# ngrabaskas/Torch-Automatic-Distributed-Neural-Network

Hardware: AMD Instinct MI355X
Metric: samples/sec whole-node ResNet-50 DP + GPT-2 PP at 1/2/4/8 MI355X; scaling eff (higher is better)
Workload: dtype bf16

## Files before the change

### madnn/ops/csrc/stem.hip

```cpp
#include "mfma.h"

namespace madnn {
namespace stem {

using namespace mf;

constexpr int kThreads = 256;
constexpr int kCo = 64;
constexpr int kKh = 7;
constexpr int kKp = 224;
constexpr int kSteps = kKp / 16;
constexpr int kMaxWo = 128;

struct StemArgs {
  const uint16_t* x;
  const uint16_t* w;
  uint16_t* y;
  float* stats;
  int N, H, W, Ho, Wo;
  int rows;
};

__device__ __forceinline__ int img_elem(int kh, int px, int c, int WP) { return (kh * WP + px) * 4 + c; }

template <bool STATS>
__global__ __launch_bounds__(kThreads, 2) void stem_fwd_kernel(const StemArgs a) {
  extern __shared__ __attribute__((aligned(16))) uint16_t smem[];
  const int WP = 2 * a.Wo + 6;
  const int IMG = kKh * WP * 4;
  uint16_t* img0 = smem;
  uint16_t* img1 = smem + IMG;
  char* otile = reinterpret_cast<char*>(smem + 2 * IMG);
  const int tid = threadIdx.x, wave = tid >> 6, lane = tid & 63, l32 = lane & 31, hh = lane >> 5;
  const int row_elems = a.W * 3;
  const int chunks = (row_elems + 7) / 8;
  const int PER = (kKh * chunks + kThreads - 1) / kThreads;

  for (int i = tid; i < IMG; i += kThreads) {
    img0[i] = 0;
    img1[i] = 0;
  }

  const int nb = wave & 1, pb0 = 64 * (wave >> 1);
  bf16x8 wf[kSteps];
#pragma unroll
  for (int s = 0; s < kSteps; ++s)
    wf[s] = *reinterpret_cast<const bf16x8*>(a.w + (32 * nb + l32) * kKp + 16 * s + 8 * hh);

  float ssum[8], ssq[8];
  if constexpr (STATS) {
#pragma unroll
    for (int e = 0; e < 8; ++e) ssum[e] = ssq[e] = 0.f;
  }

  u32x4 stg[4];
  auto load = [&](int row) {
    const int n = row / a.Ho, oh = row % a.Ho;
#pragma unroll
    for (int i = 0; i < 4; ++i) {
      const int c = tid + kThreads * i;
      stg[i] = u32x4{0u, 0u, 0u, 0u};
      if (i < PER && c < kKh * chunks) {
        const int kh = c / chunks, ch = c % chunks;
        const int ih = 2 * oh - 3 + kh;
        if (ih >= 0 && ih < a.H) {
          stg[i] = *reinterpret_cast<const u32x4*>(a.x + ((int64_t)n * a.H + ih) * row_elems + ch * 8);
        }
      }
    }
  };
  auto store = [&](uint16_t* img) {
#pragma unroll
    for (int i = 0; i < 4; ++i) {
      const int c = tid + kThreads * i;
      if (i < PER && c < kKh * chunks) {
        const int kh = c / chunks, ch = c % chunks;
#pragma unroll
        for (int k = 0; k < 8; ++k) {
          const int e = ch * 8 + k;
          const unsigned v = (stg[i][k >> 1] >> (16 * (k & 1))) & 0xffffu;
          img[img_elem(kh, e / 3 + 3, e % 3, WP)] = (uint16_t)v;
        }
      }
    }
  };

  int row = blockIdx.x;
  if (row >= a.rows) return;
  __syncthreads();
  load(row);
  store(img0);
  __syncthreads();
  int cur = 0;
  for (;;) {
    const int nrow = row + gridDim.x;
    const bool more = nrow < a.rows;
    if (more) load(nrow);
    const uint16_t* img = cur ? img1 : img0;
    f32x16 acc[2] = {zero16(), zero16()};
    if (pb0 < a.Wo) {
#pragma unroll
      for (int kh = 0; kh < kKh; ++kh)
#pragma unroll
        for (int s2 = 0; s2 < 2; ++s2) {
#pragma unroll
          for (int q = 0; q < 2; ++q) {
            const int pix = min(pb0 + 32 * q + l32, a.Wo - 1);
            const int px = 2 * pix + 4 * s2 + 2 * hh;
            const bf16x8 bx = *reinterpret_cast<const bf16x8*>(img + img_elem(kh, px, 0, WP));
            acc[q] = mfma(wf[2 * kh + s2], bx, acc[q]);
          }
        }
    }
#pragma unroll
    for (int q = 0; q < 2; ++q) {
      const int pix = pb0 + 32 * q + l32;
#pragma unroll
      for (int g = 0; g < 4; ++g) {
        const int co = 32 * nb + 8 * g + 4 * hh;
        const unsigned lo = (unsigned)f32_to_bf16(acc[q][4 * g]) | ((unsigned)f32_to_bf16(acc[q][4 * g + 1]) << 16);
        const unsigned hi = (unsigned)f32_to_bf16(acc[q][4 * g + 2]) | ((unsigned)f32_to_bf16(acc[q][4 * g + 3]) << 16);
        *reinterpret_cast<u32x2*>(otile + pix * 128 + 16 * ((co >> 3) ^ ((pix >> 1) & 7)) + 8 * ((co >> 2) & 1)) =
            u32x2{lo, hi};
      }
    }
    __syncthreads();
    {
      uint16_t* yrow = a.y + (int64_t)row * a.Wo * kCo;
      const int c = tid & 7;
      for (int r = tid >> 3; r < a.Wo; r += kThreads / 8) {
        const u32x4 v = *reinterpret_cast<const u32x4*>(otile + r * 128 + 16 * (c ^ ((r >> 1) & 7)));
        *reinterpret_cast<u32x4*>(yrow + r * kCo + 8 * c) = v;
        if constexpr (STATS) {
#pragma unroll
          for (int e = 0; e < 4; ++e) {
            const float x0 = bf16_to_f32((unsigned short)(v[e] & 0xffffu));
            const float x1 = bf16_to_f32((unsigned short)(v[e] >> 16));
            ssum[2 * e] += x0;
            ssq[2 * e] += x0 * x0;
            ssum[2 * e + 1] += x1;
            ssq[2 * e + 1] += x1 * x1;
          }
        }
      }
    }
    if (!more) break;
    store(cur ? img0 : img1);
    __syncthreads();
    cur ^= 1;
    row = nrow;
  }

  if constexpr (STATS) {
    __syncthreads();
    float* red = reinterpret_cast<float*>(otile);
    const int c = tid & 7, rg = tid >> 3;
#pragma unroll
    for (int e = 0; e < 8; ++e) {
      red[(rg * 2) * kCo + 8 * c + e] = ssum[e];
      red[(rg * 2 + 1) * kCo + 8 * c + e] = ssq[e];
    }
    __syncthreads();
    if (tid < 2 * kCo) {
      const int which = tid / kCo, co = tid % kCo;
      float v = 0.f;
      for (int g = 0; g < kThreads / 8; ++g) v += red[(g * 2 + which) * kCo + co];
      a.stats[((int64_t)blockIdx.x * 2 + which) * kCo + co] = v;
    }
  }
}

inline int stem_grid(int rows) { return rows < 2 * kNumCU ? rows : 2 * kNumCU; }

constexpr int kWMaxTiles = 4;

struct StemWArgs {
  const uint16_t* x;
  const uint16_t* dy;
  float* ws;
  int N, H, W, Ho, Wo;
  int rows, per;
  const uint16_t* y;
  const uint16_t* dp;
  const uint64_t* arg;
  const float* sc;
  const float* sh;
  const float* ca;
  const float* cb;
  const float* cc;
  int Hp, Wp, p;
};

__device__ __forceinline__ bf16x8 lds_patch(const uint16_t* img_row, int ow0, int lane) {
  const int g = lane >> 4, i = lane & 15;
  const int kw = 4 * (g & 1) + (i & 3);
  const int ow = ow0 + 8 * (g >> 1) + (i >> 2);
  typedef __attribute__((address_space(3))) s16x4 lds_s16x4;
  const uint16_t* p = img_row + (2 * ow + kw) * 4;
  const s16x4 lo = __builtin_amdgcn_ds_read_tr16_b64_v4i16((lds_s16x4*)p);
  const s16x4 hi = __builtin_amdgcn_ds_read_tr16_b64_v4i16((lds_s16x4*)(p + 8 * 4));
  const s16x8 r = {lo[0], lo[1], lo[2], lo[3], hi[0], hi[1], hi[2], hi[3]};
  return __builtin_bit_cast(bf16x8, r);
}

template <bool BNP>
__global__ __launch_bounds__(kThreads, 2) void stem_wgrad_kernel(const StemWArgs a) {
  extern __shared__ __attribute__((aligned(16))) uint16_t smem[];
  const int WOP = (a.Wo + 15) & ~15;
  const int ROW = (2 * WOP + 6) * 4;
  uint16_t* ring = smem;
  uint16_t* dyt = smem + 9 * ROW;
  const int pchunks = BNP ? a.Wp * 8 : 0;
  uint16_t* pdp = dyt + WOP * kCo;
  uint64_t* parg = reinterpret_cast<uint64_t*>(pdp + 2 * pchunks * 8);
  float* cf = reinterpret_cast<float*>(parg + 2 * pchunks);
  int tid = threadIdx.x;
  const int wave = tid >> 6, lane = tid & 63, hh = lane >> 5, l32 = lane & 31;
  const int row_elems = a.W * 3, chunks = row_elems / 8;
  const int dchunks = a.Wo * 8;

  const int r0 = blockIdx.x * a.per;
  const int r1 = min(r0 + a.per, a.rows);
  if (r0 >= r1) return;
  for (int i = tid; i < 9 * ROW + WOP * kCo; i += kThreads) smem[i] = 0;

  const int b = wave & 1, kh0 = wave >> 1;
  f32x16 acc[kWMaxTiles];
#pragma unroll
  for (int q = 0; q < kWMaxTiles; ++q) acc[q] = zero16();

  u32x4 istg[4], dstg[4];
  int s_oh = 0, s_klo = 0;
  u32x4 pstg[2];
  u32x2 astg[2];
  int s_pslot = -1;
  auto pload = [&](int n, int ohp) {
    if constexpr (BNP) asm volatile("" : "+v"(tid));
    s_pslot = ohp & 1;
    const int64_t base = ((int64_t)n * a.Hp + ohp) * pchunks;
#pragma unroll
    for (int i = 0; i < 2; ++i) {
      const int c = tid + kThreads * i;
      if (c < pchunks) {
        pstg[i] = *reinterpret_cast<const u32x4*>(a.dp + (base + c) * 8);
        astg[i] = *reinterpret_cast<const u32x2*>(a.arg + base + c);
      }
    }
  };
  auto pstore = [&]() {
    if (s_pslot < 0) return;
    if constexpr (BNP) asm volatile("" : "+v"(tid));
#pragma unroll
    for (int i = 0; i < 2; ++i) {
      const int c = tid + kThreads * i;
      if (c < pchunks) {
        *reinterpret_cast<u32x4*>(pdp + (s_pslot * pchunks + c) * 8) = pstg[i];
        *reinterpret_cast<u32x2*>(parg + s_pslot * pchunks + c) = astg[i];
      }
    }
  };
  auto load = [&](int r) {
    if constexpr (BNP) asm volatile("" : "+v"(tid));
    const int n = r / a.Ho, oh = r % a.Ho;
    const bool fresh = (r == r0) || (oh == 0);
    s_oh = oh;
    s_klo = fresh ? 0 : 5;
    if constexpr (BNP) {
      const int h1 = (oh + a.p) >> 1;
      s_pslot = -1;
      if ((fresh || ((oh + a.p) & 1) == 0) && h1 < a.Hp) pload(n, h1);
    }
    const int total = (kKh - s_klo) * chunks;
#pragma unroll
    for (int i = 0; i < 4; ++i) {
      const int c = tid + kThreads * i;
      istg[i] = u32x4{0u, 0u, 0u, 0u};
      if (c < total) {
        const int ih = 2 * oh - 3 + s_klo + c / chunks;
        if (ih >= 0 && ih < a.H)
          istg[i] = *reinterpret_cast<const u32x4*>(a.x + ((int64_t)n * a.H + ih) * row_elems + (c % chunks) * 8);
      }
      const int d = tid + kThreads * i;
      if (d < dchunks)
        dstg[i] = *reinterpret_cast<const u32x4*>((BNP ? a.y : a.dy) + ((int64_t)r * a.Wo) * kCo + d * 8);
    }
  };
  auto store = [&]() {
    if constexpr (BNP) asm volatile("" : "+v"(tid));
    const int total = (kKh - s_klo) * chunks;
#pragma unroll
    for (int i = 0; i < 4; ++i) {
      const int c = tid + kThreads * i;
      if (c < total) {
        const int ih = 2 * s_oh - 3 + s_klo + c / chunks, ch = c % chunks;
        if (ih >= 0 && ih < a.H) {
          uint16_t* img = ring + (ih & 7) * ROW;
#pragma unroll
          for (int k = 0; k < 8; ++k) {
            const int e = ch * 8 + k;
            img[(e / 3 + 3) * 4 + e % 3] = (uint16_t)((istg[i][k >> 1] >> (16 * (k & 1))) & 0xffffu);
          }
        }
      }
      if constexpr (!BNP) {
        const int d = tid + kThreads * i;
        if (d < dchunks)
          *reinterpret_cast<u32x4*>(reinterpret_cast<char*>(dyt) + swz<64>(d >> 3, d & 7)) = dstg[i];
      }
    }
    if constexpr (BNP) pstore();
  };
  auto build = [&]() {
    const int hp = s_oh + a.p, h1 = hp >> 1, hodd = hp & 1;
    const bool okh[2] = {hodd == 0 && h1 >= 1, h1 < a.Hp};
    if constexpr (BNP) asm volatile("" : "+v"(tid));
    const int cg = tid & 7;
    float v[5][8];
#pragma unroll
    for (int k = 0; k < 5; ++k) {
      const f32x4 lo = *reinterpret_cast<const f32x4*>(cf + k * kCo + cg * 8);
      const f32x4 hi = *reinterpret_cast<const f32x4*>(cf + k * kCo + cg * 8 + 4);
      v[k][0] = lo.x; v[k][1] = lo.y; v[k][2] = lo.z; v[k][3] = lo.w;
      v[k][4] = hi.x; v[k][5] = hi.y; v[k][6] = hi.z; v[k][7] = hi.w;
    }
#pragma unroll
    for (int i = 0; i < 4; ++i) {
      const int d = tid + kThreads * i;
      if (d < dchunks) {
        const int wp = (d >> 3) + a.p, w1 = wp >> 1, wodd = wp & 1;
        const bool okw[2] = {wodd == 0 && w1 >= 1, w1 < a.Wp};
        u32x4 g[4];
        u32x2 pk[4];
        bool ok[4];
        unsigned pos[4];
#pragma unroll
        for (int q = 0; q < 4; ++q) {
          const int ih = q >> 1, iw = q & 1;
          ok[q] = okh[ih] && okw[iw];
          pos[q] = (unsigned)((ih ? hodd : 2) * 3 + (iw ? wodd : 2));
          const int ow = min(max(w1 - 1 + iw, 0), a.Wp - 1);
          const int c = (((h1 - 1 + ih) & 1) * a.Wp + ow) * 8 + cg;
          g[q] = *reinterpret_cast<const u32x4*>(pdp + c * 8);
          pk[q] = *reinterpret_cast<const u32x2*>(parg + c);
        }
        u32x4 o4;
#pragma unroll
        for (int j2 = 0; j2 < 4; ++j2) {
          unsigned short ob[2];
#pragma unroll
          for (int e = 0; e < 2; ++e) {
            const int j = 2 * j2 + e;
            float acc = 0.f;
#pragma unroll
            for (int q = 0; q < 4; ++q) {
              const float gj = bf16_to_f32((unsigned short)((g[q][j >> 1] >> (16 * (j & 1))) & 0xffffu));
              const unsigned byte = (pk[q][j >> 2] >> (8 * (j & 3))) & 0xffu;
              if (ok[q]) acc += (byte == pos[q]) ? gj : 0.f;
            }
            const float yv = bf16_to_f32((unsigned short)((dstg[i][j >> 1] >> (16 * (j & 1))) & 0xffffu));
            const float z = yv * v[0][j] + v[1][j];
            acc = z > 0.f ? acc : 0.f;
            ob[e] = f32_to_bf16(v[2][j] * acc + v[3][j] * yv + v[4][j]);
          }
          o4[j2] = (unsigned)ob[0] | ((unsigned)ob[1] << 16);
        }
        *reinterpret_cast<u32x4*>(reinterpret_cast<char*>(dyt) + swz<64>(d >> 3, d & 7)) = o4;
      }
      __builtin_amdgcn_sched_barrier(0);
    }
  };

  if constexpr (BNP) {
    for (int i = tid; i < 5 * kCo; i += kThreads) {
      const float* src = i < kCo ? a.sc : i < 2 * kCo ? a.sh : i < 3 * kCo ? a.ca : i < 4 * kCo ? a.cb : a.cc;
      cf[i] = src[i % kCo];
    }
  }
  __syncthreads();
  if constexpr (BNP) {
    const int n = r0 / a.Ho, hp = r0 % a.Ho + a.p;
    if ((hp & 1) == 0 && (hp >> 1) >= 1) {
      pload(n, (hp >> 1) - 1);
      pstore();
    }
  }
  load(r0);
  store();
  __syncthreads();
  if constexpr (BNP) {
    build();
    __syncthreads();
  }
  for (int r = r0;;) {
    const int oh = r % a.Ho;
    const bool more = r + 1 < r1;
    if (more) load(r + 1);
    const uint16_t* rows_kh[kWMaxTiles];
#pragma unroll
    for (int q = 0; q < kWMaxTiles; ++q) {
      const int ih = 2 * oh - 3 + kh0 + 2 * q;
      rows_kh[q] = ring + ((ih >= 0 && ih < a.H) ? (ih & 7) : 8) * ROW;
    }
    for (int t = 0; t < WOP; t += 16) {
      const bf16x8 af = lds_col<64>(dyt, t, 32 * b, lane);
#pragma unroll
      for (int q = 0; q < kWMaxTiles; ++q)
        if (kh0 + 2 * q < kKh) acc[q] = mfma(af, lds_patch(rows_kh[q], t, lane), acc[q]);
    }
    if (!more) break;
    __syncthreads();
    store();
    __syncthreads();
    if constexpr (BNP) {
      build();
      __syncthreads();
    }
    ++r;
  }

  const int kw = l32 >> 2, c = l32 & 3;
  if (kw < 7 && c < 3) {
    float* out = a.ws + (int64_t)blockIdx.x * kCo * 147;
#pragma unroll
    for (int q = 0; q < kWMaxTiles; ++q) {
      const int kh = kh0 + 2 * q;
      if (kh < kKh) {
#pragma unroll
        for (int e = 0; e < 16; ++e) {
          const int co = 32 * b + acc_row(e, hh);
          out[co * 147 + c * 49 + kh * 7 + kw] = acc[q][e];
        }
      }
    }
  }
}

__global__ __launch_bounds__(256) void stem_wgrad_reduce(const float* __restrict__ ws, float* __restrict__ dw, int parts) {
  __shared__ float red[8][32];
  const int col = threadIdx.x & 31, grp = threadIdx.x >> 5;
  const int i = blockIdx.x * 32 + col;
  const int64_t stride = (int64_t)kCo * 147;
  float s[8] = {0.f, 0.f, 0.f, 0.f, 0.f, 0.f, 0.f, 0.f};
  if (i < kCo * 147) {
    int g = grp;
    for (; g + 56 < parts; g += 64) {
#pragma unroll
      for (int u = 0; u < 8; ++u) s[u] += ws[(int64_t)(g + 8 * u) * stride + i];
    }
    for (; g < parts; g += 8) s[0] += ws[(int64_t)g * stride + i];
  }
  red[grp][col] = ((s[0] + s[1]) + (s[2] + s[3])) + ((s[4] + s[5]) + (s[6] + s[7]));
  __syncthreads();
  if (grp == 0 && i < kCo * 147) {
    float t = 0.f;
#pragma unroll
    for (int k = 0; k < 8; ++k) t += red[k][col];
    dw[i] = t;
  }
}

inline int wgrad_grid(int rows) { return rows < 2 * kNumCU ? rows : 2 * kNumCU; }

}
}

using namespace madnn::stem;

extern "C" {

int madnn_stem_supported(int H, int W) {
  const int Wo = (W + 6 - 7) / 2 + 1;
  return (H >= 7 && W >= 8 && W % 8 == 0 && Wo <= kMaxWo && kKh * (W * 3 / 8) <= 4 * kThreads) ? 1 : 0;
}

int madnn_stem_stat_rows(int N, int H, int W) {
  const int Ho = (H + 6 - 7) / 2 + 1;
  return stem_grid(N * Ho);
}

hipError_t madnn_stem_fwd(const void* x, const void* wp, void* y, float* stats, int N, int H, int W, hipStream_t s) {
  if (!madnn_stem_supported(H, W)) return hipErrorInvalidValue;
  StemArgs a{};
  a.x = static_cast<const uint16_t*>(x);
  a.w = static_cast<const uint16_t*>(wp);
  a.y = static_cast<uint16_t*>(y);
  a.stats = stats;
  a.N = N;
  a.H = H;
  a.W = W;
  a.Ho = (H + 6 - 7) / 2 + 1;
  a.Wo = (W + 6 - 7) / 2 + 1;
  a.rows = N * a.Ho;
  if (a.rows <= 0) return hipSuccess;
  const int WP = 2 * a.Wo + 6;
  const size_t lds = (size_t)2 * kKh * WP * 4 * sizeof(uint16_t) + (size_t)kMaxWo * kCo * sizeof(uint16_t);
  const int grid = stem_grid(a.rows);
  if (stats) {
    hipLaunchKernelGGL(stem_fwd_kernel<true>, dim3(grid), dim3(kThreads), lds, s, a);
  } else {
    hipLaunchKernelGGL(stem_fwd_kernel<false>, dim3(grid), dim3(kThreads), lds, s, a);
  }
  return hipGetLastError();
}

int64_t madnn_stem_wgrad_ws(int N, int H, int W) {
  const int Ho = (H + 6 - 7) / 2 + 1;
  return (int64_t)wgrad_grid(N * Ho) * kCo * 147;
}

hipError_t madnn_stem_wgrad(const void* x, const void* dy, float* ws, float* dw, int N, int H, int W,
                            hipStream_t s) {
  if (!madnn_stem_supported(H, W)) return hipErrorInvalidValue;
  StemWArgs a{};
  a.x = static_cast<const uint16_t*>(x);
  a.dy = static_cast<const uint16_t*>(dy);
  a.ws = ws;
  a.N = N;
  a.H = H;
  a.W = W;
  a.Ho = (H + 6 - 7) / 2 + 1;
  a.Wo = (W + 6 - 7) / 2 + 1;
  a.rows = N * a.Ho;
  if (a.rows <= 0) return hipMemsetAsync(dw, 0, sizeof(float) * kCo * 147, s);
  a.per = (a.rows + wgrad_grid(a.rows) - 1) / wgrad_grid(a.rows);
  const int grid = (a.rows + a.per - 1) / a.per;
  const int WOP = (a.Wo + 15) & ~15;
  const size_t lds = (size_t)(9 * (2 * WOP + 6) * 4 + WOP * kCo) * sizeof(uint16_t);
  hipLaunchKernelGGL(stem_wgrad_kernel<false>, dim3(grid), dim3(kThreads), lds, s, a);
  MADNN_HIP_CHECK(hipGetLastError());
  hipLaunchKernelGGL(stem_wgrad_reduce, dim3((kCo * 147 + 31) / 32), dim3(256), 0, s, ws, dw, grid);
  return hipGetLastError();
}

hipError_t madnn_stem_wgrad_bnp(const void* x, const void* y, const void* dp, const void* arg, const float* scale,
                                const float* shift, const float* ca, const float* cb, const float* cc, float* ws,
                                float* dw, int N, int H, int W, int p, hipStream_t s) {
  if (!madnn_stem_supported(H, W) || p < 0 || p > 1) return hipErrorInvalidValue;
  StemWArgs a{};
  a.x = static_cast<const uint16_t*>(x);
  a.y = static_cast<const uint16_t*>(y);
  a.dp = static_cast<const uint16_t*>(dp);
  a.arg = static_cast<const uint64_t*>(arg);
  a.sc = scale;
  a.sh = shift;
  a.ca = ca;
  a.cb = cb;
  a.cc = cc;
  a.ws = ws;
  a.N = N;
  a.H = H;
  a.W = W;
  a.Ho = (H + 6 - 7) / 2 + 1;
  a.Wo = (W + 6 - 7) / 2 + 1;
  a.p = p;
  a.Hp = (a.Ho + 2 * p - 3) / 2 + 1;
  a.Wp = (a.Wo + 2 * p - 3) / 2 + 1;
  if (a.Ho + 2 * p < 3 || a.Wo + 2 * p < 3) return hipErrorInvalidValue;
  a.rows = N * a.Ho;
  if (a.rows <= 0) return hipMemsetAsync(dw, 0, sizeof(float) * kCo * 147, s);
  a.per = (a.rows + wgrad_grid(a.rows) - 1) / wgrad_grid(a.rows);
  const int grid = (a.rows + a.per - 1) / a.per;
  const int WOP = (a.Wo + 15) & ~15;
  const size_t lds = (size_t)(9 * (2 * WOP + 6) * 4 + WOP * kCo) * sizeof(uint16_t) + (size_t)2 * a.Wp * kCo * 3 +
                     5 * kCo * sizeof(float);
  hipLaunchKernelGGL(stem_wgrad_kernel<true>, dim3(grid), dim3(kThreads), lds, s, a);
  MADNN_HIP_CHECK(hipGetLastError());
  hipLaunchKernelGGL(stem_wgrad_reduce, dim3((kCo * 147 + 31) / 32), dim3(256), 0, s, ws, dw, grid);
  return hipGetLastError();
}

}
```

Baseline: 14220.

## Double-buffer stem wgrad dy tile and interleave BN/pool backward build with MFMA loop

Result: no change. 14250, median of 2 (+0.2%).

```diff
diff --git a/madnn/ops/csrc/stem.hip b/madnn/ops/csrc/stem.hip
--- a/madnn/ops/csrc/stem.hip
+++ b/madnn/ops/csrc/stem.hip
@@ -1,3 +1,5 @@
+#include <type_traits>
+
 #include "mfma.h"
 
 namespace madnn {
@@ -210,8 +212,9 @@
   const int ROW = (2 * WOP + 6) * 4;
   uint16_t* ring = smem;
   uint16_t* dyt = smem + 9 * ROW;
+  constexpr int kTiles = BNP ? 2 : 1;
   const int pchunks = BNP ? a.Wp * 8 : 0;
-  uint16_t* pdp = dyt + WOP * kCo;
+  uint16_t* pdp = dyt + kTiles * WOP * kCo;
   uint64_t* parg = reinterpret_cast<uint64_t*>(pdp + 2 * pchunks * 8);
   float* cf = reinterpret_cast<float*>(parg + 2 * pchunks);
   int tid = threadIdx.x;
@@ -222,7 +225,7 @@
   const int r0 = blockIdx.x * a.per;
   const int r1 = min(r0 + a.per, a.rows);
   if (r0 >= r1) return;
-  for (int i = tid; i < 9 * ROW + WOP * kCo; i += kThreads) smem[i] = 0;
+  for (int i = tid; i < 9 * ROW + kTiles * WOP * kCo; i += kThreads) smem[i] = 0;
 
   const int b = wave & 1, kh0 = wave >> 1;
   f32x16 acc[kWMaxTiles];
@@ -234,6 +237,10 @@
   u32x4 pstg[2];
   u32x2 astg[2];
   int s_pslot = -1;
+  auto dchunk = [&](int i) {
+    if constexpr (BNP) return ((32 * i + 2 * ((tid >> 3) & 15) + (((tid >> 7) + i) & 1)) << 3) | (tid & 7);
+    else return tid + kThreads * i;
+  };
   auto pload = [&](int n, int ohp) {
     if constexpr (BNP) asm volatile("" : "+v"(tid));
     s_pslot = ohp & 1;
@@ -259,30 +266,41 @@
       }
     }
   };
-  auto load = [&](int r) {
+  auto pload_row = [&](int r) {
+    const int n = r / a.Ho, oh = r % a.Ho;
+    const bool fresh = (r == r0) || (oh == 0);
+    const int h1 = (oh + a.p) >> 1;
+    s_pslot = -1;
+    if ((fresh || ((oh + a.p) & 1) == 0) && h1 < a.Hp) pload(n, h1);
+  };
+  auto load_x = [&](int n, int oh, int total, int i) {
+    const int c = tid + kThreads * i;
+    istg[i] = u32x4{0u, 0u, 0u, 0u};
+    if (c < total) {
+      const int ih = 2 * oh - 3 + s_klo + c / chunks;
+      if (ih >= 0 && ih < a.H)
+        istg[i] = *reinterpret_cast<const u32x4*>(a.x + ((int64_t)n * a.H + ih) * row_elems + (c % chunks) * 8);
+    }
+  };
+  auto load_y = [&](int r, int i) {
+    const int d = dchunk(i);
+    if (d < dchunks)
+      dstg[i] = *reinterpret_cast<const u32x4*>((BNP ? a.y : a.dy) + ((int64_t)r * a.Wo) * kCo + d * 8);
+  };
+  auto load = [&](int r, bool with_y) {
     if constexpr (BNP) asm volatile("" : "+v"(tid));
     const int n = r / a.Ho, oh = r % a.Ho;
     const bool fresh = (r == r0) || (oh == 0);
     s_oh = oh;
     s_klo = fresh ? 0 : 5;
     if constexpr (BNP) {
-      const int h1 = (oh + a.p) >> 1;
-      s_pslot = -1;
-      if ((fresh || ((oh + a.p) & 1) == 0) && h1 < a.Hp) pload(n, h1);
+      if (with_y) pload_row(r);
     }
     const int total = (kKh - s_klo) * chunks;
 #pragma unroll
     for (int i = 0; i < 4; ++i) {
-      const int c = tid + kThreads * i;
-      istg[i] = u32x4{0u, 0u, 0u, 0u};
-      if (c < total) {
-        const int ih = 2 * oh - 3 + s_klo + c / chunks;
-        if (ih >= 0 && ih < a.H)
-          istg[i] = *reinterpret_cast<const u32x4*>(a.x + ((int64_t)n * a.H + ih) * row_elems + (c % chunks) * 8);
-      }
-      const int d = tid + kThreads * i;
-      if (d < dchunks)
-        dstg[i] = *reinterpret_cast<const u32x4*>((BNP ? a.y : a.dy) + ((int64_t)r * a.Wo) * kCo + d * 8);
+      load_x(n, oh, total, i);
+      if (with_y) load_y(r, i);
     }
   };
   auto store = [&]() {
@@ -310,62 +328,94 @@
     }
     if constexpr (BNP) pstore();
   };
-  auto build = [&]() {
-    const int hp = s_oh + a.p, h1 = hp >> 1, hodd = hp & 1;
-    const bool okh[2] = {hodd == 0 && h1 >= 1, h1 < a.Hp};
+  const int b_wpar = __builtin_amdgcn_readfirstlane(wave >> 1) + a.p;
+  int b_h1 = 0, b_hodd = 0;
+  bool b_up = false, b_lo = false;
+  float bv[5][8];
+  auto build_begin = [&]() {
+    const int hp = s_oh + a.p;
+    b_h1 = hp >> 1;
+    b_hodd = hp & 1;
+    b_up = b_hodd == 0 && b_h1 >= 1;
+    b_lo = b_h1 < a.Hp;
     if constexpr (BNP) asm volatile("" : "+v"(tid));
     const int cg = tid & 7;
-    float v[5][8];
 #pragma unroll
     for (int k = 0; k < 5; ++k) {
       const f32x4 lo = *reinterpret_cast<const f32x4*>(cf + k * kCo + cg * 8);
       const f32x4 hi = *reinterpret_cast<const f32x4*>(cf + k * kCo + cg * 8 + 4);
-      v[k][0] = lo.x; v[k][1] = lo.y; v[k][2] = lo.z; v[k][3] = lo.w;
-      v[k][4] = hi.x; v[k][5] = hi.y; v[k][6] = hi.z; v[k][7] = hi.w;
-    }
-#pragma unroll
-    for (int i = 0; i < 4; ++i) {
-      const int d = tid + kThreads * i;
-      if (d < dchunks) {
-        const int wp = (d >> 3) + a.p, w1 = wp >> 1, wodd = wp & 1;
-        const bool okw[2] = {wodd == 0 && w1 >= 1, w1 < a.Wp};
-        u32x4 g[4];
-        u32x2 pk[4];
-        bool ok[4];
-        unsigned pos[4];
-#pragma unroll
-        for (int q = 0; q < 4; ++q) {
+      bv[k][0] = lo.x; bv[k][1] = lo.y; bv[k][2] = lo.z; bv[k][3] = lo.w;
+      bv[k][4] = hi.x; bv[k][5] = hi.y; bv[k][6] = hi.z; bv[k][7] = hi.w;
+    }
+  };
+  auto build_chunk_for = [&](int i, uint16_t* tile, auto up, auto left) {
+    constexpr bool live[4] = {decltype(up)::value && decltype(left)::value, decltype(up)::value,
+                              decltype(left)::value, true};
+    if constexpr (BNP) asm volatile("" : "+v"(tid));
+    const int cg = tid & 7;
+    const int d = dchunk(i);
+    if (d < dchunks) {
+      const int wp = (d >> 3) + a.p, w1 = wp >> 1, wodd = wp & 1;
+      const bool okh[2] = {b_up, b_lo};
+      const bool okw[2] = {wodd == 0 && w1 >= 1, w1 < a.Wp};
+      const bool ok[4] = {okh[0] && okw[0], okh[0] && okw[1], okh[1] && okw[0], okh[1] && okw[1]};
+      u32x4 g[4];
+      u32x2 pk[4];
+      unsigned pos[4];
+#pragma unroll
+      for (int q = 0; q < 4; ++q) {
+        if (live[q]) {
           const int ih = q >> 1, iw = q & 1;
-          ok[q] = okh[ih] && okw[iw];
-          pos[q] = (unsigned)((ih ? hodd : 2) * 3 + (iw ? wodd : 2));
+          pos[q] = ok[q] ? (unsigned)((ih ? b_hodd : 2) * 3 + (iw ? wodd : 2)) : 0x100u;
           const int ow = min(max(w1 - 1 + iw, 0), a.Wp - 1);
-          const int c = (((h1 - 1 + ih) & 1) * a.Wp + ow) * 8 + cg;
+          const int c = (((b_h1 - 1 + ih) & 1) * a.Wp + ow) * 8 + cg;
           g[q] = *reinterpret_cast<const u32x4*>(pdp + c * 8);
           pk[q] = *reinterpret_cast<const u32x2*>(parg + c);
         }
-        u32x4 o4;
-#pragma unroll
-        for (int j2 = 0; j2 < 4; ++j2) {
-          unsigned short ob[2];
-#pragma unroll
-          for (int e = 0; e < 2; ++e) {
-            const int j = 2 * j2 + e;
-            float acc = 0.f;
-#pragma unroll
-            for (int q = 0; q < 4; ++q) {
+      }
+      u32x4 o4;
+#pragma unroll
+      for (int j2 = 0; j2 < 4; ++j2) {
+        unsigned short ob[2];
+#pragma unroll
+        for (int e = 0; e < 2; ++e) {
+          const int j = 2 * j2 + e;
+          float acc = 0.f;
+#pragma unroll
+          for (int q = 0; q < 4; ++q) {
+            if (live[q]) {
               const float gj = bf16_to_f32((unsigned short)((g[q][j >> 1] >> (16 * (j & 1))) & 0xffffu));
               const unsigned byte = (pk[q][j >> 2] >> (8 * (j & 3))) & 0xffu;
-              if (ok[q]) acc += (byte == pos[q]) ? gj : 0.f;
+              acc += (byte == pos[q]) ? gj : 0.f;
             }
-            const float yv = bf16_to_f32((unsigned short)((dstg[i][j >> 1] >> (16 * (j & 1))) & 0xffffu));
-            const float z = yv * v[0][j] + v[1][j];
-            acc = z > 0.f ? acc : 0.f;
-            ob[e] = f32_to_bf16(v[2][j] * acc + v[3][j] * yv + v[4][j]);
           }
-          o4[j2] = (unsigned)ob[0] | ((unsigned)ob[1] << 16);
-        }
-        *reinterpret_cast<u32x4*>(reinterpret_cast<char*>(dyt) + swz<64>(d >> 3, d & 7)) = o4;
-      }
+          const float yv = bf16_to_f32((unsigned short)((dstg[i][j >> 1] >> (16 * (j & 1))) & 0xffffu));
+          const float z = __builtin_fmaf(yv, bv[0][j], bv[1][j]);
+          acc = z > 0.f ? acc : 0.f;
+          ob[e] = f32_to_bf16(__builtin_fmaf(bv[3][j], yv, bv[2][j] * acc) + bv[4][j]);
+        }
+        o4[j2] = (unsigned)ob[0] | ((unsigned)ob[1] << 16);
+      }
+      *reinterpret_cast<u32x4*>(reinterpret_cast<char*>(tile) + swz<64>(d >> 3, d & 7)) = o4;
+    }
+  };
+  using yes = std::integral_constant<bool, true>;
+  using no = std::integral_constant<bool, false>;
+  auto build_chunk = [&](int i, uint16_t* tile) {
+    const bool b_left = ((b_wpar + i) & 1) == 0;
+    if (b_up) {
+      if (b_left) build_chunk_for(i, tile, yes{}, yes{});
+      else build_chunk_for(i, tile, yes{}, no{});
+    } else {
+      if (b_left) build_chunk_for(i, tile, no{}, yes{});
+      else build_chunk_for(i, tile, no{}, no{});
+    }
+  };
+  auto build = [&]() {
+    build_begin();
+#pragma unroll
+    for (int i = 0; i < 4; ++i) {
+      build_chunk_for(i, dyt, yes{}, yes{});
       __builtin_amdgcn_sched_barrier(0);
     }
   };
@@ -384,38 +434,83 @@
       pstore();
     }
   }
-  load(r0);
+  load(r0, true);
   store();
   __syncthreads();
   if constexpr (BNP) {
     build();
+    if (r0 + 1 < r1) {
+      __syncthreads();
+      asm volatile("" : "+v"(tid));
+      pload_row(r0 + 1);
+      pstore();
+#pragma unroll
+      for (int i = 0; i < 4; ++i) load_y(r0 + 1, i);
+    }
     __syncthreads();
-  }
-  for (int r = r0;;) {
-    const int oh = r % a.Ho;
-    const bool more = r + 1 < r1;
-    if (more) load(r + 1);
-    const uint16_t* rows_kh[kWMaxTiles];
-#pragma unroll
-    for (int q = 0; q < kWMaxTiles; ++q) {
-      const int ih = 2 * oh - 3 + kh0 + 2 * q;
-      rows_kh[q] = ring + ((ih >= 0 && ih < a.H) ? (ih & 7) : 8) * ROW;
-    }
-    for (int t = 0; t < WOP; t += 16) {
-      const bf16x8 af = lds_col<64>(dyt, t, 32 * b, lane);
-#pragma unroll
-      for (int q = 0; q < kWMaxTiles; ++q)
-        if (kh0 + 2 * q < kKh) acc[q] = mfma(af, lds_patch(rows_kh[q], t, lane), acc[q]);
-    }
-    if (!more) break;
-    __syncthreads();
-    store();
-    __syncthreads();
-    if constexpr (BNP) {
-      build();
+    const int nt = WOP / 16;
+    int cur = 0;
+    for (int r = r0;;) {
+      const int oh = r % a.Ho;
+      const bool more = r + 1 < r1, more2 = r + 2 < r1;
+      s_pslot = -1;
+      if (more) {
+        load(r + 1, false);
+        if (more2) pload_row(r + 2);
+        build_begin();
+      }
+      const uint16_t* rows_kh[kWMaxTiles];
+#pragma unroll
+      for (int q = 0; q < kWMaxTiles; ++q) {
+        const int ih = 2 * oh - 3 + kh0 + 2 * q;
+        rows_kh[q] = ring + ((kh0 + 2 * q < kKh && ih >= 0 && ih < a.H) ? (ih & 7) : 8) * ROW;
+      }
+      const uint16_t* ta = dyt + cur * WOP * kCo;
+      uint16_t* tb = dyt + (cur ^ 1) * WOP * kCo;
+      for (int ti = 0; ti < nt; ++ti) {
+        const bf16x8 af = lds_col<64>(ta, 16 * ti, 32 * b, lane);
+#pragma unroll
+        for (int q = 0; q < kWMaxTiles; ++q) acc[q] = mfma(af, lds_patch(rows_kh[q], 16 * ti, lane), acc[q]);
+        if (more) {
+#pragma unroll
+          for (int i = 0; i < 4; ++i) {
+            if (i * nt / 4 == ti) {
+              build_chunk(i, tb);
+              if (more2) load_y(r + 2, i);
+            }
+          }
+        }
+      }
+      if (!more) break;
       __syncthreads();
-    }
-    ++r;
+      store();
+      __syncthreads();
+      cur ^= 1;
+      ++r;
+    }
+  } else {
+    for (int r = r0;;) {
+      const int oh = r % a.Ho;
+      const bool more = r + 1 < r1;
+      if (more) load(r + 1, true);
+      const uint16_t* rows_kh[kWMaxTiles];
+#pragma unroll
+      for (int q = 0; q < kWMaxTiles; ++q) {
+        const int ih = 2 * oh - 3 + kh0 + 2 * q;
+        rows_kh[q] = ring + ((ih >= 0 && ih < a.H) ? (ih & 7) : 8) * ROW;
+      }
+      for (int t = 0; t < WOP; t += 16) {
+        const bf16x8 af = lds_col<64>(dyt, t, 32 * b, lane);
+#pragma unroll
+        for (int q = 0; q < kWMaxTiles; ++q)
+          if (kh0 + 2 * q < kKh) acc[q] = mfma(af, lds_patch(rows_kh[q], t, lane), acc[q]);
+      }
+      if (!more) break;
+      __syncthreads();
+      store();
+      __syncthreads();
+      ++r;
+    }
   }
 
   const int kw = l32 >> 2, c = l32 & 3;
@@ -561,7 +656,7 @@
   a.per = (a.rows + wgrad_grid(a.rows) - 1) / wgrad_grid(a.rows);
   const int grid = (a.rows + a.per - 1) / a.per;
   const int WOP = (a.Wo + 15) & ~15;
-  const size_t lds = (size_t)(9 * (2 * WOP + 6) * 4 + WOP * kCo) * sizeof(uint16_t) + (size_t)2 * a.Wp * kCo * 3 +
+  const size_t lds = (size_t)(9 * (2 * WOP + 6) * 4 + 2 * WOP * kCo) * sizeof(uint16_t) + (size_t)2 * a.Wp * kCo * 3 +
                      5 * kCo * sizeof(float);
   hipLaunchKernelGGL(stem_wgrad_kernel<true>, dim3(grid), dim3(kThreads), lds, s, a);
   MADNN_HIP_CHECK(hipGetLastError());
```
